# manuelbb-upb/Morbit.jl

Hardware: AMD Instinct MI355X
Metric: RBF build+solve+eval cycles/sec (higher is better)
Workload: dtype f64

## Files before the change

### morbit.jl_amd/csrc/backsolve.hip

```cpp
#include "common.hpp"

namespace mrbf {

namespace bsolve {

constexpr int NB = 128, NTHR = 512;
typedef double v2d __attribute__((ext_vector_type(2)));
typedef double v4d __attribute__((ext_vector_type(4)));
typedef __attribute__((address_space(1))) unsigned gu32;
typedef __attribute__((address_space(1))) double gf64;
typedef __attribute__((address_space(1))) v2d gv2d;

template <int KB>
struct Shared {
    double xs[2][KB][NB];
    int ok;
};

__global__ __launch_bounds__(256) void premul_kernel(const double *__restrict__ L, int64_t lda, const double *__restrict__ linv_all,
                                                     double *__restrict__ Mbuf, int nb, unsigned *__restrict__ flags, int nflags,
                                                     unsigned long long *__restrict__ xb, int nxb) {
    for (int e = blockIdx.x * 256 + threadIdx.x; e < nflags; e += gridDim.x * 256) flags[e] = 0u;
    for (int e = blockIdx.x * 256 + threadIdx.x; e < nxb; e += gridDim.x * 256) xb[e] = ~0ull;
    const int slab = blockIdx.x & 3, t = (blockIdx.x >> 2) & 1, j = blockIdx.x >> 3;
    const int i = j + 1 + t;
    if (i >= nb) return;
    const double *A = L + (int64_t)i * NB + (int64_t)j * NB * lda;
    const double *B = linv_all + (size_t)j * NB * NB;
    double *M = Mbuf + ((size_t)j * 2 + t) * NB * NB;
    const int lane = threadIdx.x & 63, wave = threadIdx.x >> 6, l15 = lane & 15, l4 = lane >> 4;
    const int i0 = 32 * wave, j0 = 32 * slab;
    v4d acc[2][2];
#pragma unroll
    for (int a = 0; a < 2; ++a)
#pragma unroll
        for (int b = 0; b < 2; ++b) acc[a][b] = (v4d){0.0, 0.0, 0.0, 0.0};
    const double *pa = A + (i0 + l15) + (int64_t)(j0 + l4) * lda;
    const double *pb = B + (j0 + l4) + (int64_t)(j0 + l15) * NB;
    constexpr int UK = 8;
    double fa0[2][UK], fa1[2][UK], fb0[2][UK], fb1[2][UK];
    auto burst = [&](int buf) {
#pragma unroll
        for (int u = 0; u < UK; ++u) {
            fa0[buf][u] = pa[(int64_t)4 * u * lda];
            fa1[buf][u] = pa[(int64_t)4 * u * lda + 16];
            fb0[buf][u] = pb[4 * u];
            fb1[buf][u] = pb[4 * u + 16 * NB];
        }
        pa += (int64_t)4 * UK * lda;
        pb += 4 * UK;
    };
    auto mma = [&](int buf) {
#pragma unroll
        for (int u = 0; u < UK; ++u) {
            acc[0][0] = __builtin_amdgcn_mfma_f64_16x16x4f64(fa0[buf][u], fb0[buf][u], acc[0][0], 0, 0, 0);
            acc[0][1] = __builtin_amdgcn_mfma_f64_16x16x4f64(fa0[buf][u], fb1[buf][u], acc[0][1], 0, 0, 0);
            acc[1][0] = __builtin_amdgcn_mfma_f64_16x16x4f64(fa1[buf][u], fb0[buf][u], acc[1][0], 0, 0, 0);
            acc[1][1] = __builtin_amdgcn_mfma_f64_16x16x4f64(fa1[buf][u], fb1[buf][u], acc[1][1], 0, 0, 0);
        }
    };
    const int nburst = (NB - j0) / (4 * UK);
    burst(0);
    for (int b = 0; b < nburst; b += 2) {
        if (b + 1 < nburst) burst(1);
        mma(0);
        if (b + 1 >= nburst) break;
        if (b + 2 < nburst) burst(0);
        mma(1);
    }
#pragma unroll
    for (int a = 0; a < 2; ++a)
#pragma unroll
        for (int b = 0; b < 2; ++b)
#pragma unroll
            for (int r = 0; r < 4; ++r) M[(i0 + 16 * a + l4 + 4 * r) + (size_t)(j0 + 16 * b + l15) * NB] = acc[a][b][r];
}

__device__ __forceinline__ void load_tile(const double *__restrict__ T, int64_t ldt, v2d (&r)[2][8]) {
    const int lane = threadIdx.x & 63, w = threadIdx.x >> 6;
    const double *p = T + (int64_t)(16 * w + 2 * (lane >> 3)) * ldt + 2 * (lane & 7);
#pragma unroll
    for (int cc = 0; cc < 2; ++cc)
#pragma unroll
        for (int u = 0; u < 8; ++u) r[cc][u] = *(const gv2d *)(p + cc * ldt + 16 * u);
}

template <int N>
__device__ __forceinline__ double shl_lanes(double v) {
    const long long b = __double_as_longlong(v);
    const int lo = __builtin_amdgcn_update_dpp((int)b, (int)b, 0x100 + N, 0xf, 0xf, false);
    const int hi = __builtin_amdgcn_update_dpp((int)(b >> 32), (int)(b >> 32), 0x100 + N, 0xf, 0xf, false);
    return __longlong_as_double(((long long)hi << 32) | (unsigned)lo);
}

template <int KB>
__device__ __forceinline__ void tile_dot(const double (*xs)[NB], const v2d (&r)[2][8], double (&out)[2][KB]) {
    const int q = threadIdx.x & 7;
    double acc[2][KB];
#pragma unroll
    for (int cc = 0; cc < 2; ++cc)
#pragma unroll
        for (int l = 0; l < KB; ++l) acc[cc][l] = 0.0;
#pragma unroll
    for (int u = 0; u < 8; ++u) {
#pragma unroll
        for (int l = 0; l < KB; ++l) {
            const v2d x = *(const v2d *)&xs[l][16 * u + 2 * q];
#pragma unroll
// ... 202 lines not shown
    double last[2][KB];
#pragma unroll
    for (int cc = 0; cc < 2; ++cc)
#pragma unroll
        for (int l = 0; l < KB; ++l) last[cc][l] = 0.0;
    if (npm >= 1) {
        if (stamps && tid == 0) stamps[256 * 4 + j] = (long long)wall_clock64();
        await_block<KB>(sh, sh.xs[1], xb, j + 1, fillv, 0, abortw, epoch, spin_ticks, status, 0x700);
        if (stamps && tid == 0) stamps[j * 4 + 0] = (long long)wall_clock64();
        lds_barrier();
        if (!sh.ok) return;
        if (stamps && tid == 0) stamps[j * 4 + 1] = (long long)wall_clock64();
        tile_dot<KB>(sh.xs[1], tm1, last);
    } else {
        lds_barrier();
        if (!sh.ok) return;
    }
    if ((fault & 1) && j == nb / 2) return;
    if (stamps && tid == 0) stamps[j * 4 + 2] = (long long)wall_clock64();
    if (q == 0) {
#pragma unroll
        for (int l = 0; l < KB; ++l) {
            const v2d v = (v2d){(zj[l][0] - acc[0][l]) - last[0][l], (zj[l][1] - acc[1][l]) - last[1][l]};
            publish(&xb[((size_t)j * KB + l) * NB + col], v);
            *(v2d *)&Y[(int64_t)(k0 + l) * ldy + (int64_t)j * NB + col] = v;
        }
    }
}

}

int backsolve_blocked(mrbf_ctx *ctx, int64_t npad, const double *L, int64_t lda, const double *linv_all, double *Y, int64_t ldy, int k);

int backsolve_persistent(mrbf_ctx *ctx, int64_t npad, const double *L, int64_t lda, const double *linv_all, double *Y, int64_t ldy, int k,
                         int *status) {
    using namespace bsolve;
    const int nb = (int)(npad / NB);
    static const int force_old = mrbf_env("MRBF_BACKSOLVE_LAUNCHES") ? atoi(mrbf_env("MRBF_BACKSOLVE_LAUNCHES")) : 0;
    const int ncu = ctx->ncu;
    if (force_old || nb < 3 || nb > ncu || (lda & 1) || (reinterpret_cast<uintptr_t>(L) & 15))
        return backsolve_blocked(ctx, npad, L, lda, linv_all, Y, ldy, k);
    unsigned *flags;
    MRBF_TRY(get_buf(ctx, S_BSOLVE_FLAGS, (size_t)(nb + 1) * 32, &flags));
    const unsigned long long spin_ticks = (unsigned long long)std::max(1, ctx->spin_ms) * 100000ull;
    const int fault = (ctx->debug_fault & 2) ? 1 : 0;
    double *xb, *Mbuf;
    MRBF_TRY(get_buf(ctx, S_BSOLVE_X, (size_t)2 * nb * 4 * NB, &xb));
    MRBF_TRY(get_buf(ctx, S_BSOLVE_M, (size_t)nb * 2 * NB * NB, &Mbuf));
    hipLaunchKernelGGL(premul_kernel, dim3((unsigned)(8 * (nb - 1))), dim3(256), 0, ctx->stream, L, lda, linv_all, Mbuf, nb, flags, (nb + 1) * 32,
                       reinterpret_cast<unsigned long long *>(xb), 2 * nb * 4 * NB);
    static const bool want_stamps = mrbf_env("MRBF_BSOLVE_STAMPS") && atoi(mrbf_env("MRBF_BSOLVE_STAMPS")) != 0;
    long long *stamps = nullptr;
    if (want_stamps) {
        static long long *dbg = nullptr;
        if (!dbg) MRBF_HIP(ctx, hipMalloc(&dbg, (size_t)256 * 9 * sizeof(long long)));
        stamps = dbg;
    }
    unsigned epoch = 0;
    for (int k0 = 0; k0 < k; k0 += 4) {
        const int kb = std::min(4, k - k0);
        ++epoch;
        if (k0 > 0) MRBF_HIP(ctx, hipMemsetAsync(xb, 0xff, (size_t)2 * nb * 4 * NB * sizeof(double), ctx->stream));
#define MRBF_BSP(KBV)                                                                                                          \
    hipLaunchKernelGGL((backsolve_persistent_kernel<KBV>), dim3((unsigned)(2 * nb)), dim3(NTHR), 0, ctx->stream, L, lda, linv_all, Mbuf, Y, ldy, k0, nb, \
                       flags, epoch, spin_ticks, status, fault, xb, xb + (size_t)nb * 4 * NB, stamps)
        if (kb == 1) MRBF_BSP(1); else if (kb == 2) MRBF_BSP(2); else if (kb == 3) MRBF_BSP(3); else MRBF_BSP(4);
#undef MRBF_BSP
    }
    MRBF_HIP(ctx, hipGetLastError());
    if (want_stamps) {
        std::vector<long long> h((size_t)256 * 9);
        MRBF_HIP(ctx, hipMemcpyAsync(h.data(), stamps, h.size() * sizeof(long long), hipMemcpyDeviceToHost, ctx->stream));
        MRBF_HIP(ctx, hipStreamSynchronize(ctx->stream));
        double seen = 0, bar = 0, dot = 0, hop = 0, late = 0;
        int cnt = 0;
        for (int j = 1; j + 2 < nb; ++j) {
            seen += (double)(h[j * 4 + 0] - h[(j + 1) * 4 + 2]);
            bar += (double)(h[j * 4 + 1] - h[j * 4 + 0]);
            dot += (double)(h[j * 4 + 2] - h[j * 4 + 1]);
            hop += (double)(h[j * 4 + 2] - h[(j + 1) * 4 + 2]);
            late += (double)(h[256 * 4 + j] - h[(j + 1) * 4 + 2]);
            ++cnt;
        }
// ... 21 lines not shown
```

### morbit.jl_amd/csrc/chol_mega.hip

```cpp
#include <chrono>

#include "chol_diag_core.hpp"
#include "common.hpp"
#include "mega_gemm.hpp"

namespace mrbf {

typedef double v4d __attribute__((ext_vector_type(4)));
typedef double v2d __attribute__((ext_vector_type(2)));

namespace mega {

constexpr int WIN_DEFAULT = 4;

enum { JOB_U = 0, JOB_T = 1, JOB_P = 2, JOB_S = 3, JOB_UH = 4 };
struct Job {
    short kind, i, c, w;
};
enum { CTL_QP = 0, CTL_ABORT = 32, CTL_TIMEOUT = 64, CTL_PCOLS = 96, CTL_QC = 128, CTL_TS = 144 , CTL_WORDS = 160 };
constexpr int QSTRIDE = 32;
__host__ __device__ inline int wstart(int w, int first, int win) { return w <= 0 ? 0 : first + win * (w - 1); }
__host__ __device__ inline int nbulk_updates(int i, int c, int slack, int slack_chain, int first, int win, int srows = 2) {
    const int t = c - ((i - c <= srows) ? slack_chain : slack);
    return t < first ? 0 : (t - first) / win + 1;
}

struct Edge {
    int head, tail_c0, srows_edge, pstream_edge;
    int shalf, sh_head, sh_tail_c0;
    int tfull1;
    int xhalf;
};
__host__ __device__ inline bool edge_col(int c, const Edge &e) { return c < e.head || c >= e.tail_c0; }
__host__ __device__ inline int srows_at(int c, int srows, const Edge &e) { return edge_col(c, e) ? e.srows_edge : srows; }
__host__ __device__ inline bool shalf_at(int c, int srows, const Edge &e) { return e.shalf && (c < e.sh_head || c >= e.sh_tail_c0) && srows_at(c, srows, e) >= 5; }
__host__ __device__ inline bool tfull_at(int i, int c, int srows, const Edge &e) { return e.tfull1 > 0 && i - c - srows_at(c, srows, e) > e.tfull1 - 1; }
__host__ __device__ inline bool xhalf_at(int i, int nt, const Edge &e) { return e.xhalf && i >= nt; }

struct Args {
    double *A;
    int64_t lda;
    int NT, MT;
    double *linv;
    unsigned *tdone;
    unsigned *ucnt;
    unsigned *ctl;
    const Job *pjobs;
    int npanel;
    const Job *bjobs;
    int nbulk;
    const int *wq_start;
    unsigned *wq_head;
    double *itg;
    unsigned *dprog;
    unsigned *sprog;
    unsigned *quiet;
    int nwin;
    int *info;
    const Job *cjobs;
    int nchainjobs;
    int nchain;
    int ndedicated;
    int look;
    unsigned long long spin_ticks;
    int fault;
    int use_quiet;
    int xchain;
    int quiet_tail;
    int slack, slack_chain, first, win, wbias, srows;
    Edge edge;
    int cboost;
    int head_job1;
    int nreserve;
    int reserve_job0;
    unsigned long long *jlog;
    int jlog_cap;
    int pstream;
    int panel_dma;
    int trace_dbg;
    unsigned long long *trace;
};

struct Shared {
    union {
        double gemm[4 * 2 * 8 * LDS_LD];
        diagcore::DiagV6Shared diag;
    } u;
    int ok;
    int jkind, jidx;
    unsigned long long *jrec;
    int wlo;
    int cwlo;
    int mycu;
};

typedef __attribute__((address_space(1))) unsigned gu32;
typedef __attribute__((address_space(1))) double gf64;
__device__ __forceinline__ unsigned ldf(const unsigned *p) {
    return __hip_atomic_load((const gu32 *)p, __ATOMIC_RELAXED, __HIP_MEMORY_SCOPE_AGENT);
}
__device__ __forceinline__ void stf(unsigned *p, unsigned v) { __hip_atomic_store((gu32 *)p, v, __ATOMIC_RELAXED, __HIP_MEMORY_SCOPE_AGENT); }
__device__ __forceinline__ unsigned addf(unsigned *p, unsigned v) {
    return __hip_atomic_fetch_add((gu32 *)p, v, __ATOMIC_RELAXED, __HIP_MEMORY_SCOPE_AGENT);
}
__device__ __forceinline__ void st_sc1(double *p, double v) { __hip_atomic_store((gf64 *)p, v, __ATOMIC_RELAXED, __HIP_MEMORY_SCOPE_AGENT); }
__device__ __forceinline__ int64_t uni64(int64_t v) {
    const unsigned lo = (unsigned)__builtin_amdgcn_readfirstlane((int)(unsigned)(unsigned long long)v);
    const unsigned hi = (unsigned)__builtin_amdgcn_readfirstlane((int)(unsigned)((unsigned long long)v >> 32));
    return (int64_t)(((unsigned long long)hi << 32) | lo);
}
template <class T>
__device__ __forceinline__ T *uni_ptr(T *q) {
    return reinterpret_cast<T *>(uni64(reinterpret_cast<int64_t>(q)));
// ... 588 lines not shown
            }
        }
        if (has_mask == 0ull) {
            if (!moved) return -2;
            continue;
        }
        unsigned key = 0xffffffffu;
        if (has) {
            const Job jb = a.bjobs[base + (int)h];
            const int jw = jb.w & 255, pl = wstart(jw + 1, a.first, a.win) - 1;
            if (ldf(a.tdone + (size_t)jb.i * a.NT + pl) >= 2u && ldf(a.tdone + (size_t)jb.c * a.NT + pl) >= 2u &&
                ldf(a.ucnt + (size_t)jb.i * a.NT + jb.c) >= (unsigned)(2 * jw))
                key = ((unsigned)(1024 + jb.c + a.wbias * wnd - (cls ? a.cboost : 0)) << 8) | (unsigned)lane;
        }
        unsigned best = key;
#pragma unroll
        for (int off = 32; off > 0; off >>= 1) {
            const unsigned o = (unsigned)__shfl_xor((int)best, off);
            best = o < best ? o : best;
        }
        if (best == 0xffffffffu) return -1;
        const int win_lane = (int)(best & 0xffu);
        int got = -1;
        if (lane == win_lane) {
            const unsigned g = addf(a.wq_head + (size_t)wq * QSTRIDE, 1u);
            if (g < (unsigned)cnt) got = base + (int)g;
        }
        got = __shfl(got, win_lane);
        if (got >= 0) return got;
    }
    return -1;
}

__device__ __forceinline__ void mega_body(const Args &a) {
    __shared__ __attribute__((aligned(16))) Shared sh;
    const int bx = (int)blockIdx.x;
    const int nx = a.xchain, cls = nx > 0 && (bx & 7) < nx;
    const int cidx = !cls ? -1 : (bx < 256 ? (bx >> 3) * nx + (bx & 7) : 32 * nx + ((bx - 256) >> 3) * nx + (bx & 7));
    const int oidx = nx == 0 ? bx - a.nchain : (cls ? -1 : (bx < 256 ? bx - ((bx >> 3) * nx + nx) : bx - 32 * nx - (((bx - 256) >> 3) * nx + nx)));
    const bool chain = nx ? (cls && cidx < a.nchain) : bx < a.nchain;
    const bool dedicated = !chain && oidx >= 0 && oidx < a.ndedicated;
    if (chain || dedicated) __builtin_amdgcn_s_setprio(2);
    if (threadIdx.x == 0) {
        sh.wlo = 0;
        sh.cwlo = 0;
        const unsigned hw = __builtin_amdgcn_s_getreg((31 << 11) | 4);
        const unsigned xcc = __builtin_amdgcn_s_getreg((31 << 11) | 20);
        sh.mycu = (int)(((xcc & 7u) << 6) | (((hw >> 13) & 3u) << 4) | ((hw >> 8) & 15u));
    }
    __syncthreads();
    unsigned *myquiet = a.quiet + (size_t)sh.mycu * QSTRIDE;
    const bool reserve = !chain && cls && cidx < a.nchain + a.nreserve;
    bool in_chain = chain;
    if (reserve && threadIdx.x == 0) {
        const unsigned qc = ldf(a.ctl + CTL_QC);
        sh.jidx = (qc < (unsigned)a.head_job1 || qc >= (unsigned)a.reserve_job0) ? 1 : 0;
    }
    if (reserve) {
        __syncthreads();
        in_chain = sh.jidx != 0;
        __syncthreads();
    }
    unsigned long long idle_t0 = 0;
    int nidle = 0;
    while (true) {
    if (in_chain) {
        if (a.use_quiet && threadIdx.x == 0) addf(myquiet, 1u);
        if (reserve) __builtin_amdgcn_s_setprio(2);
        bool leave = false;
        while (true) {
            if (threadIdx.x == 0) {
                int idx = -1;
                if (!ldf(a.ctl + CTL_ABORT)) {
                    if (reserve) {
                        const unsigned qc = ldf(a.ctl + CTL_QC);
                        if (qc >= (unsigned)a.head_job1 && qc < (unsigned)a.reserve_job0) idx = -2;
                    }
                    if (idx != -2) {
                        const unsigned got = addf(a.ctl + CTL_QC, 1u);
                        if (got < (unsigned)a.nchainjobs) idx = (int)got;
                    }
                }
                sh.jidx = idx;
            }
            __syncthreads();
            const int idx = sh.jidx;
            __syncthreads();
            if (idx == -2) {
                leave = true;
                break;
            }
            if (idx < 0) break;
            const Job jb = a.cjobs[idx];
            jlog_begin(a, sh, jb);
            if (!(jb.kind == JOB_P ? (a.trace ? run_diag<true>(a, sh, jb) : run_diag<false>(a, sh, jb))
                                   : (jb.w == 0 ? run_stream<false>(a, sh, jb) : run_stream<true>(a, sh, jb))))
                break;
            jlog_end(sh);
        }
        if (a.use_quiet && threadIdx.x == 0) addf(myquiet, 0xffffffffu);
        if (!leave) return;
        __builtin_amdgcn_s_setprio(0);
        in_chain = false;
        idle_t0 = 0;
        nidle = 0;
        continue;
    }
    {
        if (threadIdx.x < 64) {
            int kind = -1, idx = 0;
            bool panel_left = false;
            if (ldf(a.ctl + CTL_ABORT)) {
                kind = -2;
            } else if (reserve && ldf(a.ctl + CTL_QC) >= (unsigned)a.reserve_job0 && ldf(a.ctl + CTL_QC) < (unsigned)a.nchainjobs) {
                kind = -3;
            } else if (!dedicated && a.use_quiet && ldf(myquiet) != 0 && a.NT - (int)ldf(a.ctl + CTL_PCOLS) <= a.quiet_tail) {
                kind = -1;
                idle_t0 = 0;
            } else {
                const unsigned ph = ldf(a.ctl + CTL_QP);
                panel_left = ph < (unsigned)a.npanel;
                bool want_panel = false;
                if (panel_left) {
                    if (dedicated || a.ndedicated == 0)
                        want_panel = true;
                    else {
                        const Job hj = a.pjobs[ph];
                        want_panel = hj.c < (int)ldf(a.ctl + CTL_PCOLS) + a.look &&
                                     ldf(a.ucnt + (size_t)hj.i * a.NT + hj.c) >=
                                         2u * (unsigned)nbulk_updates(hj.i, hj.c, a.slack, a.slack_chain, a.first, a.win, srows_at(hj.c, a.srows, a.edge));
                    }
                }
                if (want_panel) {
                    unsigned got = 0;
// ... 36 lines not shown
        __syncthreads();
        if (kind == -2) break;
        if (kind == -3) {
            in_chain = true;
            continue;
        }
        if (kind == -1) {
            ++nidle;
            const int reps = nidle < 8 ? 1 : (nidle < 32 ? 4 : 16);
            for (int r = 0; r < reps; ++r) __builtin_amdgcn_s_sleep(64);
            continue;
        }
        idle_t0 = 0;
        nidle = 0;
        bool ok;
        const unsigned long long tj0 = a.trace ? wall_clock64() : 0ull;
        jlog_begin(a, sh, kind == 1 ? a.pjobs[idx] : a.bjobs[idx]);
        if (kind == 1) {
            if (!dedicated) __builtin_amdgcn_s_setprio(1);
            ok = a.pjobs[idx].w == 2 ? run_panel<true>(a, sh, a.pjobs[idx]) : run_panel<false>(a, sh, a.pjobs[idx]);
            if (!dedicated) __builtin_amdgcn_s_setprio(0);
        } else {
            ok = a.bjobs[idx].kind == JOB_UH ? run_bulk<64>(a, sh, a.bjobs[idx]) : run_bulk<128>(a, sh, a.bjobs[idx]);
        }
        jlog_end(sh);
        if (a.trace && threadIdx.x == 0) {
            unsigned long long *u = a.trace + (size_t)a.NT * 16 + (size_t)blockIdx.x * 4;
            u[kind == 1 ? 1 : 0] += wall_clock64() - tj0;
            u[kind == 1 ? 3 : 2] += 1;
        }
        if (!ok) break;
    }
    }
}

__global__ __launch_bounds__(256, 2) void potrf_mega_kernel(const Args a) {
    if (threadIdx.x == 0)
        __hip_atomic_fetch_max((unsigned long long *)(a.ctl + CTL_TS), ~(unsigned long long)wall_clock64(), __ATOMIC_RELAXED, __HIP_MEMORY_SCOPE_AGENT);
    mega_body(a);
    if (threadIdx.x == 0)
        __hip_atomic_fetch_max((unsigned long long *)(a.ctl + CTL_TS + 2), (unsigned long long)wall_clock64(), __ATOMIC_RELAXED, __HIP_MEMORY_SCOPE_AGENT);
}

__global__ void mega_status_kernel(const unsigned *ctl, int *info, unsigned long long *stat) {
    if (ctl[CTL_TIMEOUT] != 0 && *info == 0) *info = -(int)ctl[CTL_TIMEOUT];
    const unsigned long long *ts = (const unsigned long long *)(ctl + CTL_TS);
    if (stat) stat[0] = (ts[0] != 0 && ts[1] != 0) ? ts[1] - ~ts[0] : 0ull;
}

}

static void build_job_tables(int NT, int MT, int slack, int slack_chain, int first, int win, int srows, const mega::Edge &edge, int half_cols,
                             int tail_half, int tail_half_w, bool chainq, std::vector<mega::Job> &pj, std::vector<mega::Job> &bj, std::vector<mega::Job> &cj, std::vector<int> &wqs) {
    using namespace mega;
    pj.clear();
    bj.clear();
    cj.clear();
    wqs.clear();
    for (int c = 0; c < NT; ++c) {
        cj.push_back(Job{JOB_P, (short)c, (short)c, (short)0});
        for (int i = c + 1; i < MT; ++i) {
            if (i <= c + srows_at(c, srows, edge)) {
                if (shalf_at(c, srows, edge)) {
                    cj.push_back(Job{JOB_S, (short)i, (short)c, (short)1});
                    cj.push_back(Job{JOB_S, (short)i, (short)c, (short)2});
                } else {
// ... 197 lines not shown
            if (c < NT) job += 1 + (shalf_at(c, srows, edge) ? 2 : 1) * std::min(srows_at(c, srows, edge), MT - 1 - c);
        }
        a.nreserve = (e_head > 0 || e_tail_c0 < NT) ? (env_reserve >= 0 ? env_reserve : 12) : 0;
    }
    {
        static const int env_pdma = mrbf_env("MRBF_MEGA_PANELDMA") ? atoi(mrbf_env("MRBF_MEGA_PANELDMA")) : 1;
        a.panel_dma = env_pdma;
    }
    a.pstream = ctx->mega_pstream > 0 ? std::min(ctx->mega_pstream, srows) : (NTq <= 48 && srows >= 2 ? 2 : 1);
    a.spin_ticks = (unsigned long long)std::max(1, ctx->spin_ms) * 100000ull;
    a.fault = (ctx->debug_fault & 1) && MT > 1;
    const int grid = (NT <= 16 && ctx->mega_grid > 256) ? 256 : ctx->mega_grid;
    if (a.nchain < 1) a.nchain = 1;
    if (a.nchain + a.ndedicated >= grid) a.ndedicated = std::max(0, grid / 2 - a.nchain);
    {
        static const int env_xc = mrbf_env("MRBF_MEGA_XCHAIN") ? atoi(mrbf_env("MRBF_MEGA_XCHAIN")) : -1;
        const int xc = env_xc >= 0 ? env_xc : (a.nchain > 48 ? 4 : (a.nchain > 32 ? 2 : 1));
        a.xchain = (xc > 0 && 8 * a.nchain <= std::min(xc, 8) * grid) ? std::min(xc, 8) : 0;
        static const int qt = mrbf_env("MRBF_MEGA_QUIET_TAIL") ? atoi(mrbf_env("MRBF_MEGA_QUIET_TAIL")) : -1;
        a.quiet_tail = qt >= 0 ? qt : (NTq > 96 ? 32 : 1 << 20);
    }
    const char *trace_path = mrbf_env("MRBF_MEGA_TRACE");
    if (trace_path) {
        a.trace_dbg = mrbf_env("MRBF_MEGA_TRACE_WAVE") ? 12 + 16 * (atoi(mrbf_env("MRBF_MEGA_TRACE_WAVE")) & 3) : 4;
        MRBF_TRY(get_buf(ctx, S_MEGA_TRACE, (size_t)NT * 80 + 4 * 1024, &a.trace));
        MRBF_HIP(ctx, hipMemsetAsync(a.trace, 0, ((size_t)NT * 80 + 4 * 1024) * sizeof(unsigned long long), ctx->stream));
    }
    const char *jlog_path = mrbf_env("MRBF_MEGA_JLOG");
    if (jlog_path) {
        a.jlog_cap = ctx->mega_npanel + ctx->mega_nbulk + ctx->mega_nchainjobs + 16;
        MRBF_TRY(get_buf(ctx, S_MEGA_JLOG, (size_t)8 * a.jlog_cap + 16, &a.jlog));
        MRBF_HIP(ctx, hipMemsetAsync(a.jlog, 0, ((size_t)8 * a.jlog_cap + 16) * sizeof(unsigned long long), ctx->stream));
    }
    hipLaunchKernelGGL(potrf_mega_kernel, dim3((unsigned)grid), dim3(256), 0, ctx->stream, a);
    hnow();
    if (jlog_path) {
        std::vector<unsigned long long> h((size_t)8 * a.jlog_cap + 16);
        MRBF_HIP(ctx, hipStreamSynchronize(ctx->stream));
        MRBF_HIP(ctx, hipMemcpy(h.data(), a.jlog, h.size() * sizeof(unsigned long long), hipMemcpyDeviceToHost));
        if (FILE *f = fopen(jlog_path, "w")) {
            const unsigned long long n = std::min<unsigned long long>(h[0], (unsigned long long)a.jlog_cap);
            unsigned long long t0 = ~0ull;
            for (unsigned long long j = 0; j < n; ++j) t0 = std::min(t0, h[8 + 8 * j + 1]);
            for (unsigned long long j = 0; j < n; ++j) {
                const unsigned long long *r = &h[8 + 8 * j];
                fprintf(f, "%llu %llu %llu %llu %llu", r[0] & 0xff, (r[0] >> 8) & 0xffff, (r[0] >> 24) & 0xffff, (r[0] >> 40) & 0xfff, r[0] >> 52);
                for (int k = 1; k < 8; ++k) fprintf(f, " %.2f", r[k] ? (double)(r[k] - t0) * 0.01 : -1.0);
                fprintf(f, "\n");
            }
            fclose(f);
        }
    }
    MRBF_HIP(ctx, hipGetLastError());
    if (trace_path) {
        std::vector<unsigned long long> h((size_t)NT * 2 * 8);
        MRBF_HIP(ctx, hipStreamSynchronize(ctx->stream));
        MRBF_HIP(ctx, hipMemcpy(h.data(), a.trace, h.size() * sizeof(unsigned long long), hipMemcpyDeviceToHost));
        if (FILE *f = fopen(trace_path, "w")) {
            const unsigned long long t0 = h[0];
            for (int c = 0; c < NT; ++c) {
                fprintf(f, "%d", c);
                for (int k = 0; k < 8; ++k) fprintf(f, " %.2f", h[(size_t)c * 16 + k] ? (double)(h[(size_t)c * 16 + k] - t0) * 0.01 : -1.0);
                for (int k = 8; k < 15; ++k) fprintf(f, " %.0f", (double)h[(size_t)c * 16 + k]);
                fprintf(f, " %.2f", h[(size_t)c * 16 + 15] ? (double)(h[(size_t)c * 16 + 15] - t0) * 0.01 : -1.0);
                fprintf(f, "\n");
            }
// ... 157 lines not shown
```

### morbit.jl_amd/csrc/common.hpp

```cpp
#pragma once
#include <hip/hip_runtime.h>
#include <rocblas/rocblas.h>
#include <rocsolver/rocsolver.h>

#include <cmath>
#include <cstdlib>
#include <cstdint>
#include <cstdio>
#include <cstring>
#include <map>
#include <string>
#include <vector>

#include "../../include/mrbf.h"

namespace mrbf {

struct KP {
    int kid;
    double a, b;
    double a2;
    double sgn;
    int fast;
    int ik;
// ... 30 lines not shown
    int device = 0;
    int ncu = 256;
    hipStream_t own_stream = nullptr;
    hipStream_t stream = nullptr;
    rocblas_handle blas = nullptr;
    mrbf::Buf slots[mrbf::S_NSLOTS];
    hipEvent_t ev[8] = {};
    hipStream_t panel_stream = nullptr;
    hipEvent_t evx[4] = {};
    hipStream_t bulk_stream = nullptr;
    int bulk_masked = 0;
    int bulk_grid = 384;
    int mega_nt = 0, mega_mt = 0, mega_npanel = 0, mega_nbulk = 0, mega_nwin = 0, mega_nchainjobs = 0;
    int mega_grid = 512, mega_dedicated = 64, mega_look = 2, mega_min = 256, mega_max = 32768, mega_quiet = 1, mega_chain = 0, mega_slack = 3, mega_slack_chain = 0, mega_tab_slack = -1, mega_half_cols = 0, mega_first_window = 1, mega_win = 0, mega_wbias = 4, mega_pstream = 0, mega_srows = 0;
    std::string err;
    std::vector<mrbf::Buf> model_pool;
    int gram_mode = 0, residual = 1, force_path = 0, chol_impl = 0, eval_impl = 0, timing = 1, diag_impl = 0, chol_window = 0;
    int spin_ms = 1000, debug_fault = 0;
    unsigned long long *mega_stat_dev = nullptr;
    long mega_stat_shape = 0;
    int mega_stat_pending = 0;
    char *pin_base = nullptr;
    size_t pin_off = 0;
    bool pin_armed = false;
    struct PinOut {
        void *user;
        const void *pin;
        size_t bytes;
    };
    std::vector<PinOut> pin_out;
    unsigned long long *hpin = nullptr;
    int mega_info_clean = 0;
    int mega_xreal = 0;
    float last_device_ms = 0.f;
    int slow_launches = 0;
    int small_nc = 4;
    int small_cluster_ok = 0;
    int small_timeouts = 0;
    const double *eval_pre_xq = nullptr;
    int eval_population = 0;
    int eval_check_call = 0;
    int live_models = 0, live_round4 = 0;
    unsigned ps_rank_epoch = 0;
    int ps_multi_off = 0;
    std::map<long, float> mega_best_ms;
    std::vector<mrbf::MegaTables> mega_tables;
    unsigned long long mega_table_clock = 0;
};

struct mrbf_model {
    int64_t n = 0, npad = 0;
    int d = 0, dpad = 0, k = 0, q = 0, deg = -1;
    mrbf::KP kp{};
    double *C = nullptr;
    double *Xc = nullptr;
    double *sq = nullptr;
    double *mean = nullptr;
    double *W = nullptr;
    double *Wc = nullptr;
    double *lam = nullptr;
    void *block = nullptr;
    size_t block_bytes = 0;
};

namespace mrbf {

// ... 92 lines not shown
```

### morbit.jl_amd/csrc/solve.hip

```cpp
#include "common.hpp"
#include "small.hpp"

namespace mrbf {

__global__ void fit_publish_kernel(const int *__restrict__ dinfo, const double *__restrict__ scal, const unsigned long long *__restrict__ dstat,
                                   int *__restrict__ hflags, double *__restrict__ hscal, unsigned long long *__restrict__ hstat) {
    const int t = threadIdx.x;
    if (t < 4) hflags[t] = dinfo[t];
    if (t >= 4 && t < 6 && scal) hscal[t - 4] = scal[t - 4];
    if (t == 6 && dstat && hstat) hstat[0] = dstat[0];
}

__global__ void fill_saddle_kernel(const double *__restrict__ Pi, int64_t n, int q, double *__restrict__ S, int64_t N) {
    const int64_t idx = (int64_t)blockIdx.x * blockDim.x + threadIdx.x;
    const int64_t tot = n * q;
    if (idx < tot) {
        const int64_t i = idx % n;
        const int t = (int)(idx / n);
        const double v = Pi[idx];
        S[i + (n + t) * N] = v;
        S[(n + t) + i * N] = v;
    } else if (idx < tot + (int64_t)q * q) {
        const int64_t r = idx - tot;
        S[(n + r % q) + (n + r / q) * N] = 0.0;
// ... 239 lines not shown
    hipLaunchKernelGGL(rhs_from_values_kernel, dim3(nblk(N * k)), dim3(256), 0, ctx->stream, Y, n, k, B, N);
    MRBF_HIP(ctx, hipEventRecord(ctx->ev[0], ctx->stream));
    MRBF_TRY(launch_gram(ctx, ctx->gram_mode, M->C, M->Xc, M->sq, n, M->npad, M->d, M->dpad, M->kp, S, N));
    MRBF_HIP(ctx, hipEventRecord(ctx->ev[1], ctx->stream));
    MRBF_TRY(launch_poly_matrix(ctx, M->C, n, M->d, q, Pi, n));
    hipLaunchKernelGGL(fill_saddle_kernel, dim3(nblk(n * q + (int64_t)q * q)), dim3(256), 0, ctx->stream, Pi, n, q, S, N);
    MRBF_HIP(ctx, hipGetLastError());
    MRBF_BLAS(ctx, rocsolver_dgesvd(ctx->blas, rocblas_svect_all, rocblas_svect_all, (int)N, (int)N, S, (int)N, sv, U, (int)N, VT,
                                    (int)N, E, rocblas_outofplace, dinfo));
    MRBF_HIP(ctx, hipEventRecord(ctx->ev[2], ctx->stream));
    int hinfo = 0;
    MRBF_TRY(read_info(ctx, dinfo, &hinfo));
    info->factor_info = hinfo;
    info->path = MRBF_PATH_MINNORM;
    if (hinfo != 0) return fail(ctx, MRBF_ESINGULAR, "SVD of the saddle matrix did not converge (info = %d)", hinfo);
    MRBF_BLAS(ctx, rocblas_dgemm(ctx->blas, rocblas_operation_transpose, rocblas_operation_none, (int)N, k, (int)N, &one, U, (int)N,
                                 B, (int)N, &zero, T, (int)N));
    hipLaunchKernelGGL(scale_rows_pinv_kernel, dim3(nblk(N * k)), dim3(256), 0, ctx->stream, T, (int)N, k, sv);
    MRBF_BLAS(ctx, rocblas_dgemm(ctx->blas, rocblas_operation_transpose, rocblas_operation_none, (int)N, k, (int)N, &one, VT, (int)N,
                                 T, (int)N, &zero, B, (int)N));
    hipLaunchKernelGGL(scatter_solution_kernel, dim3(nblk(M->npad * k + (int64_t)q * k)), dim3(256), 0, ctx->stream, B, N, n,
                       M->npad, k, q, n, M->W, M->Wc, M->lam, B, N);
    MRBF_HIP(ctx, hipGetLastError());
    MRBF_HIP(ctx, hipEventRecord(ctx->ev[3], ctx->stream));
    MRBF_HIP(ctx, hipEventSynchronize(ctx->ev[3]));
    MRBF_HIP(ctx, hipEventElapsedTime(&info->ms_gram, ctx->ev[0], ctx->ev[1]));
    MRBF_HIP(ctx, hipEventElapsedTime(&info->ms_factor, ctx->ev[1], ctx->ev[2]));
    MRBF_HIP(ctx, hipEventElapsedTime(&info->ms_solve, ctx->ev[2], ctx->ev[3]));
    return 0;
}

int potrf_blocked_tall(mrbf_ctx *ctx, int64_t ncols, int64_t mrows, double *A, int64_t lda, int *dinfo, double *linv_all);
int backsolve_blocked(mrbf_ctx *ctx, int64_t npad, const double *L, int64_t lda, const double *linv_all, double *Y, int64_t ldy, int k);
int backsolve_persistent(mrbf_ctx *ctx, int64_t npad, const double *L, int64_t lda, const double *linv_all, double *Y, int64_t ldy, int k,
                         int *status);
int launch_update_lower(mrbf_ctx *ctx, const double *A, int64_t lda, const double *B, int64_t ldb, double *C, int64_t ldc, int64_t nt, int K,
                        const double *cvec, double cs, int64_t cn);
int launch_pad_identity(mrbf_ctx *ctx, double *A, int64_t n, int64_t npad, int64_t ld);
int tsmm_tn(mrbf_ctx *ctx, int64_t n, int p, int r, double alpha, const double *A, int64_t lda, const double *B, int64_t ldb, double beta,
            double *C, int64_t ldc);
int symm_panel(mrbf_ctx *ctx, int64_t n, int64_t npad, int q, const double *Phi, int64_t ld, const double *Q, int64_t ldq, double *W,
               int64_t ldwo, bool const_first, double cval);

__global__ void set_rhs_rows_kernel(double *__restrict__ A, int64_t ld, int64_t npad, int xt, const double *__restrict__ B, int k) {
    const int64_t idx = (int64_t)blockIdx.x * blockDim.x + threadIdx.x;
    if (idx >= npad * xt) return;
    const int l = (int)(idx % xt);
    const int64_t i = idx / xt;
    A[(npad + l) + i * ld] = (l < k) ? B[i + (int64_t)l * npad] : 0.0;
}
__global__ void get_rhs_rows_kernel(const double *__restrict__ A, int64_t ld, int64_t npad, double *__restrict__ B, int k) {
    const int64_t idx = (int64_t)blockIdx.x * blockDim.x + threadIdx.x;
    if (idx >= npad * k) return;
    const int l = (int)(idx % k);
    const int64_t i = idx / k;
    B[i + (int64_t)l * npad] = A[(npad + l) + i * ld];
}
__global__ void xc_to_tall_kernel(const double *__restrict__ Xc, int64_t n, int d, int dpad, double *__restrict__ Tall, int64_t lt,
                                  int64_t dq) {
    const int64_t idx = (int64_t)blockIdx.x * blockDim.x + threadIdx.x;
    if (idx >= n * d) return;
    const int64_t i = idx / d;
    const int t = (int)(idx % d);
    Tall[(dq + i) + (int64_t)t * lt] = Xc[i * dpad + t];
}
__global__ void build_q1_kernel(const double *__restrict__ Tall, int64_t lt, int64_t dq, int64_t n, int64_t npad, int q,
// ... 325 lines not shown
        const int K2 = (int)round_up(2 * (q - skip), 16);
        double *PA, *PB, *v0 = nullptr;
        MRBF_TRY(get_buf(ctx, S_STAGE_C, (size_t)npad * K2, &PA));
        MRBF_TRY(get_buf(ctx, S_STAGE_D, (size_t)npad * K2, &PB));
        if (skip) MRBF_TRY(get_buf(ctx, S_V0, (size_t)npad, &v0));
        MRBF_TRY(launch_projection_small(ctx, M, Wpart, rspart, nseg, LxInv, Q1, Wm, G, scal, dinfo, K2, skip, PA, PB, v0));
        MRBF_TRY(launch_update_lower(ctx, PA, npad, PB, npad, Phi, ld, npad / 128, K2, v0, 1.0 / std::sqrt((double)n), n));
    } else if (q > 0) {
        MRBF_TRY(symm_panel(ctx, n, npad, q, Phi, ld, Q1, npad, Wm, npad, true, 1.0 / std::sqrt((double)n)));
        MRBF_TRY(tsmm_tn(ctx, n, q, q, 1.0, Q1, npad, Wm, npad, 0.0, G, q));
        hipLaunchKernelGGL(trace_kernel, dim3(1), dim3(256), 0, ctx->stream, G, q, scal);
        MRBF_BLAS(ctx, rocblas_dgemm(ctx->blas, rocblas_operation_none, rocblas_operation_none, (int)n, q, q, &mhalf, Q1, (int)npad,
                                     G, q, &one, Wm, (int)npad));
        hipLaunchKernelGGL(shift_from_trace_kernel, dim3(1), dim3(1), 0, ctx->stream, scal, (double)n * M->kp.phi0,
                           (double)std::max<int64_t>(n - q, 1), dinfo);
        const int skip = (q > 1 && round_up(2 * (q - 1), 16) < round_up(2 * q, 16)) ? 1 : 0;
        const int K2 = (int)round_up(2 * (q - skip), 16);
        double *PA, *PB, *v0 = nullptr;
        MRBF_TRY(get_buf(ctx, S_STAGE_C, (size_t)npad * K2, &PA));
        MRBF_TRY(get_buf(ctx, S_STAGE_D, (size_t)npad * K2, &PB));
        if (skip) MRBF_TRY(get_buf(ctx, S_V0, (size_t)npad, &v0));
        hipLaunchKernelGGL(build_panels_kernel, dim3(nblk(npad * K2)), dim3(256), 0, ctx->stream, Q1, Wm, scal, n, npad, q, K2, skip, PA, PB, v0);
        MRBF_TRY(launch_update_lower(ctx, PA, npad, PB, npad, Phi, ld, npad / 128, K2, v0, 1.0 / std::sqrt((double)n), n));
    }
    MRBF_HIP(ctx, hipEventRecord(ctx->ev[2], ctx->stream));
    int hinfo = 0;
    double *linv_all = nullptr;
    if (builtin) {
        MRBF_TRY(get_buf(ctx, S_CHOL_WS, (size_t)npad * 128, &linv_all));
        MRBF_TRY(launch_pad_identity(ctx, Phi, n, npad, ld));
        if (q == 0) hipLaunchKernelGGL(set_rhs_rows_kernel, dim3(nblk(npad * xt)), dim3(256), 0, ctx->stream, Phi, ld, npad, xt, B, k);
        ctx->mega_xreal = k;
        ctx->mega_info_clean = 1;
        const int rc_potrf = potrf_blocked_tall(ctx, npad, npad + xt, Phi, ld, dinfo, linv_all);
        ctx->mega_xreal = 0;
        ctx->mega_info_clean = 0;
        if (rc_potrf != 0) return rc_potrf;
        MRBF_HIP(ctx, hipEventRecord(ctx->ev[3], ctx->stream));
    } else {
        int *dpot;
        MRBF_TRY(get_buf(ctx, S_IPIV, (size_t)4, &dpot));
        MRBF_BLAS(ctx, rocsolver_dpotrf(ctx->blas, rocblas_fill_lower, (int)n, Phi, (int)ld, dpot));
        MRBF_HIP(ctx, hipMemcpyAsync(dinfo, dpot, sizeof(int), hipMemcpyDeviceToDevice, ctx->stream));
        MRBF_HIP(ctx, hipEventRecord(ctx->ev[3], ctx->stream));
    }
    double *T1w = nullptr;
    if (q > 0) MRBF_TRY(get_buf(ctx, S_T1W, (size_t)q * k, &T1w));
    auto solve_tail = [&](bool persistent) -> int {
        if (builtin) {
            hipLaunchKernelGGL(get_rhs_rows_kernel, dim3(nblk(npad * k)), dim3(256), 0, ctx->stream, Phi, ld, npad, B, k);
            if (persistent)
                MRBF_TRY(backsolve_persistent(ctx, npad, Phi, ld, linv_all, B, npad, k, dinfo + 3));
            else
                MRBF_TRY(backsolve_blocked(ctx, npad, Phi, ld, linv_all, B, npad, k));
        } else {
            MRBF_BLAS(ctx, rocsolver_dpotrs(ctx->blas, rocblas_fill_lower, (int)n, k, Phi, (int)ld, B, (int)npad));
        }
        static const int tail3 = mrbf_env("MRBF_TAIL3") ? atoi(mrbf_env("MRBF_TAIL3")) : 1;
        if (tail3 && q > 0 && q <= 129 && k <= 16 && (q == 1 || LxInv)) {
            const int nch = (int)(npad / 64);
            double *T2, *part;
            MRBF_TRY(get_buf(ctx, S_T2, (size_t)q * k, &T2));
            MRBF_TRY(get_buf(ctx, S_TAIL_PART, (size_t)nch * 2 * k * q, &part));
            hipLaunchKernelGGL(tail_dots_kernel, dim3((unsigned)nch), dim3(256), 0, ctx->stream, B, npad, Q1, Wm, npad, n, q, k, part);
            hipLaunchKernelGGL(tail_coeff_kernel, dim3(1), dim3(1024), 0, ctx->stream, part, nch, q, k, q > 1 ? d : 0, T1, G, fused ? 1.0 : 0.5, LxInv,
                               std::sqrt((double)n), M->mean, T2, T1w);
            hipLaunchKernelGGL(tail_apply_kernel, dim3((unsigned)nch), dim3(256), 0, ctx->stream, B, npad, Q1, npad, T2, T1w, n, M->npad, q, k, M->W,
// ... 323 lines not shown
```

Measured before the change: 177.4.

## Fold backsolve premultiply jobs into the persistent Cholesky mega kernel

Moves the off-diagonal L·Linv premultiply tiles that the persistent backsolve needs into the tail of the Cholesky mega kernel. Workgroups claim jobs through an atomic counter once the needed tiles are marked done. Chain-exiting groups may wait on those readiness flags, while idle groups only take jobs that are already ready. The backsolve then skips its separate premul launch when the request was served. This removes a kernel launch and overlaps the premultiply with Cholesky tail work. The cost is extra request and done state in the context, extra spin-waiting inside the mega kernel, and a limit to NT of 16 or less.

```diff
diff --git a/morbit.jl_amd/csrc/backsolve.hip b/morbit.jl_amd/csrc/backsolve.hip
--- a/morbit.jl_amd/csrc/backsolve.hip
+++ b/morbit.jl_amd/csrc/backsolve.hip
@@ -1,4 +1,5 @@
 #include "common.hpp"
+#include "premul.hpp"
 
 namespace mrbf {
 
@@ -20,60 +21,7 @@
 __global__ __launch_bounds__(256) void premul_kernel(const double *__restrict__ L, int64_t lda, const double *__restrict__ linv_all,
                                                      double *__restrict__ Mbuf, int nb, unsigned *__restrict__ flags, int nflags,
                                                      unsigned long long *__restrict__ xb, int nxb) {
-    for (int e = blockIdx.x * 256 + threadIdx.x; e < nflags; e += gridDim.x * 256) flags[e] = 0u;
-    for (int e = blockIdx.x * 256 + threadIdx.x; e < nxb; e += gridDim.x * 256) xb[e] = ~0ull;
-    const int slab = blockIdx.x & 3, t = (blockIdx.x >> 2) & 1, j = blockIdx.x >> 3;
-    const int i = j + 1 + t;
-    if (i >= nb) return;
-    const double *A = L + (int64_t)i * NB + (int64_t)j * NB * lda;
-    const double *B = linv_all + (size_t)j * NB * NB;
-    double *M = Mbuf + ((size_t)j * 2 + t) * NB * NB;
-    const int lane = threadIdx.x & 63, wave = threadIdx.x >> 6, l15 = lane & 15, l4 = lane >> 4;
-    const int i0 = 32 * wave, j0 = 32 * slab;
-    v4d acc[2][2];
-#pragma unroll
-    for (int a = 0; a < 2; ++a)
-#pragma unroll
-        for (int b = 0; b < 2; ++b) acc[a][b] = (v4d){0.0, 0.0, 0.0, 0.0};
-    const double *pa = A + (i0 + l15) + (int64_t)(j0 + l4) * lda;
-    const double *pb = B + (j0 + l4) + (int64_t)(j0 + l15) * NB;
-    constexpr int UK = 8;
-    double fa0[2][UK], fa1[2][UK], fb0[2][UK], fb1[2][UK];
-    auto burst = [&](int buf) {
-#pragma unroll
-        for (int u = 0; u < UK; ++u) {
-            fa0[buf][u] = pa[(int64_t)4 * u * lda];
-            fa1[buf][u] = pa[(int64_t)4 * u * lda + 16];
-            fb0[buf][u] = pb[4 * u];
-            fb1[buf][u] = pb[4 * u + 16 * NB];
-        }
-        pa += (int64_t)4 * UK * lda;
-        pb += 4 * UK;
-    };
-    auto mma = [&](int buf) {
-#pragma unroll
-        for (int u = 0; u < UK; ++u) {
-            acc[0][0] = __builtin_amdgcn_mfma_f64_16x16x4f64(fa0[buf][u], fb0[buf][u], acc[0][0], 0, 0, 0);
-            acc[0][1] = __builtin_amdgcn_mfma_f64_16x16x4f64(fa0[buf][u], fb1[buf][u], acc[0][1], 0, 0, 0);
-            acc[1][0] = __builtin_amdgcn_mfma_f64_16x16x4f64(fa1[buf][u], fb0[buf][u], acc[1][0], 0, 0, 0);
-            acc[1][1] = __builtin_amdgcn_mfma_f64_16x16x4f64(fa1[buf][u], fb1[buf][u], acc[1][1], 0, 0, 0);
-        }
-    };
-    const int nburst = (NB - j0) / (4 * UK);
-    burst(0);
-    for (int b = 0; b < nburst; b += 2) {
-        if (b + 1 < nburst) burst(1);
-        mma(0);
-        if (b + 1 >= nburst) break;
-        if (b + 2 < nburst) burst(0);
-        mma(1);
-    }
-#pragma unroll
-    for (int a = 0; a < 2; ++a)
-#pragma unroll
-        for (int b = 0; b < 2; ++b)
-#pragma unroll
-            for (int r = 0; r < 4; ++r) M[(i0 + 16 * a + l4 + 4 * r) + (size_t)(j0 + 16 * b + l15) * NB] = acc[a][b][r];
+    premul::premul_job((int)blockIdx.x, L, lda, linv_all, Mbuf, nb, flags, nflags, xb, nxb, [](int, int) { return true; });
 }
 
 __device__ __forceinline__ void load_tile(const double *__restrict__ T, int64_t ldt, v2d (&r)[2][8]) {
@@ -342,23 +290,54 @@
 
 int backsolve_blocked(mrbf_ctx *ctx, int64_t npad, const double *L, int64_t lda, const double *linv_all, double *Y, int64_t ldy, int k);
 
+namespace bsolve {
+static bool persistent_path(mrbf_ctx *ctx, int nb, const double *L, int64_t lda) {
+    static const int force_old = mrbf_env("MRBF_BACKSOLVE_LAUNCHES") ? atoi(mrbf_env("MRBF_BACKSOLVE_LAUNCHES")) : 0;
+    return !(force_old || nb < 3 || nb > ctx->ncu || (lda & 1) || (reinterpret_cast<uintptr_t>(L) & 15));
+}
+static int buffers(mrbf_ctx *ctx, int nb, unsigned **flags, double **xb, double **Mbuf) {
+    MRBF_TRY(get_buf(ctx, S_BSOLVE_FLAGS, (size_t)(nb + 1) * 32, flags));
+    MRBF_TRY(get_buf(ctx, S_BSOLVE_X, (size_t)2 * nb * 4 * NB, xb));
+    MRBF_TRY(get_buf(ctx, S_BSOLVE_M, (size_t)nb * 2 * NB * NB, Mbuf));
+    return 0;
+}
+}
+
+int bsolve_premul_request(mrbf_ctx *ctx, int64_t npad, const double *L, int64_t lda, const double *linv_all) {
+    using namespace bsolve;
+    ctx->premul_req = mrbf_ctx::PremulReq{};
+    ctx->premul_done = mrbf_ctx::PremulReq{};
+    static const int env_on = mrbf_env("MRBF_MEGA_PREMUL") ? atoi(mrbf_env("MRBF_MEGA_PREMUL")) : 1;
+    const int nb = (int)(npad / NB);
+    if (!env_on || !linv_all || !persistent_path(ctx, nb, L, lda)) return 0;
+    mrbf_ctx::PremulReq r;
+    double *xb;
+    MRBF_TRY(buffers(ctx, nb, &r.flags, &xb, &r.M));
+    r.xb = reinterpret_cast<unsigned long long *>(xb);
+    r.L = L;
+    r.linv = linv_all;
+    r.lda = lda;
+    r.nb = nb;
+    ctx->premul_req = r;
+    return 0;
+}
+
 int backsolve_persistent(mrbf_ctx *ctx, int64_t npad, const double *L, int64_t lda, const double *linv_all, double *Y, int64_t ldy, int k,
                          int *status) {
     using namespace bsolve;
     const int nb = (int)(npad / NB);
-    static const int force_old = mrbf_env("MRBF_BACKSOLVE_LAUNCHES") ? atoi(mrbf_env("MRBF_BACKSOLVE_LAUNCHES")) : 0;
-    const int ncu = ctx->ncu;
-    if (force_old || nb < 3 || nb > ncu || (lda & 1) || (reinterpret_cast<uintptr_t>(L) & 15))
-        return backsolve_blocked(ctx, npad, L, lda, linv_all, Y, ldy, k);
+    const mrbf_ctx::PremulReq done = ctx->premul_done;
+    ctx->premul_done = mrbf_ctx::PremulReq{};
+    if (!persistent_path(ctx, nb, L, lda)) return backsolve_blocked(ctx, npad, L, lda, linv_all, Y, ldy, k);
     unsigned *flags;
-    MRBF_TRY(get_buf(ctx, S_BSOLVE_FLAGS, (size_t)(nb + 1) * 32, &flags));
+    double *xb, *Mbuf;
+    MRBF_TRY(buffers(ctx, nb, &flags, &xb, &Mbuf));
     const unsigned long long spin_ticks = (unsigned long long)std::max(1, ctx->spin_ms) * 100000ull;
     const int fault = (ctx->debug_fault & 2) ? 1 : 0;
-    double *xb, *Mbuf;
-    MRBF_TRY(get_buf(ctx, S_BSOLVE_X, (size_t)2 * nb * 4 * NB, &xb));
-    MRBF_TRY(get_buf(ctx, S_BSOLVE_M, (size_t)nb * 2 * NB * NB, &Mbuf));
-    hipLaunchKernelGGL(premul_kernel, dim3((unsigned)(8 * (nb - 1))), dim3(256), 0, ctx->stream, L, lda, linv_all, Mbuf, nb, flags, (nb + 1) * 32,
-                       reinterpret_cast<unsigned long long *>(xb), 2 * nb * 4 * NB);
+    if (!(done.L == L && done.linv == linv_all && done.lda == lda && done.nb == nb && done.M == Mbuf && done.flags == flags &&
+          done.xb == reinterpret_cast<unsigned long long *>(xb)))
+        hipLaunchKernelGGL(premul_kernel, dim3((unsigned)(8 * (nb - 1))), dim3(256), 0, ctx->stream, L, lda, linv_all, Mbuf, nb, flags, (nb + 1) * 32,
+                           reinterpret_cast<unsigned long long *>(xb), 2 * nb * 4 * NB);
     static const bool want_stamps = mrbf_env("MRBF_BSOLVE_STAMPS") && atoi(mrbf_env("MRBF_BSOLVE_STAMPS")) != 0;
     long long *stamps = nullptr;
     if (want_stamps) {
diff --git a/morbit.jl_amd/csrc/chol_mega.hip b/morbit.jl_amd/csrc/chol_mega.hip
--- a/morbit.jl_amd/csrc/chol_mega.hip
+++ b/morbit.jl_amd/csrc/chol_mega.hip
@@ -3,6 +3,7 @@
 #include "chol_diag_core.hpp"
 #include "common.hpp"
 #include "mega_gemm.hpp"
+#include "premul.hpp"
 
 namespace mrbf {
 
@@ -17,7 +18,7 @@
 struct Job {
     short kind, i, c, w;
 };
-enum { CTL_QP = 0, CTL_ABORT = 32, CTL_TIMEOUT = 64, CTL_PCOLS = 96, CTL_QC = 128, CTL_TS = 144 , CTL_WORDS = 160 };
+enum { CTL_QP = 0, CTL_ABORT = 32, CTL_TIMEOUT = 64, CTL_PCOLS = 96, CTL_QC = 128, CTL_TS = 144 , CTL_PM = 160, CTL_WORDS = 192 };
 constexpr int QSTRIDE = 32;
 __host__ __device__ inline int wstart(int w, int first, int win) { return w <= 0 ? 0 : first + win * (w - 1); }
 __host__ __device__ inline int nbulk_updates(int i, int c, int slack, int slack_chain, int first, int win, int srows = 2) {
@@ -79,6 +80,11 @@
     int panel_dma;
     int trace_dbg;
     unsigned long long *trace;
+    double *pm_M;
+    unsigned *pm_flags;
+    int pm_nflags;
+    unsigned long long *pm_xb;
+    int pm_nxb;
 };
 
 struct Shared {
@@ -733,6 +739,35 @@
     return -1;
 }
 
+__device__ __attribute__((noinline)) void run_premul(const Args &a, Shared &sh, bool may_wait) {
+    const int njobs = 8 * (a.NT - 1);
+    while (true) {
+        if (threadIdx.x == 0) {
+            int idx = -1;
+            unsigned h = ldf(a.ctl + CTL_PM);
+            while (h < (unsigned)njobs) {
+                const int j = (int)(h >> 3), i = j + 1 + (int)((h >> 2) & 1u);
+                if (!may_wait && !ldf(a.ctl + CTL_ABORT) && i < a.NT &&
+                    !(ldf(a.tdone + (size_t)i * a.NT + j) >= 2u && ldf(a.tdone + (size_t)j * a.NT + j) >= 2u))
+                    break;
+                if (__hip_atomic_compare_exchange_strong((gu32 *)(a.ctl + CTL_PM), &h, h + 1u, __ATOMIC_RELAXED, __ATOMIC_RELAXED,
+                                                         __HIP_MEMORY_SCOPE_AGENT)) {
+                    idx = (int)h;
+                    break;
+                }
+            }
+            sh.jidx = idx;
+        }
+        __syncthreads();
+        const int b = sh.jidx;
+        __syncthreads();
+        if (b < 0) return;
+        premul::premul_job(b, a.A, a.lda, a.linv, a.pm_M, a.NT, a.pm_flags, a.pm_nflags, a.pm_xb, a.pm_nxb, [&](int i, int j) {
+            return wg_wait(sh, a, a.tdone + (size_t)i * a.NT + j, 2u, a.tdone + (size_t)j * a.NT + j, 2u, nullptr, 0, 0x800u);
+        });
+    }
+}
+
 __device__ __forceinline__ void mega_body(const Args &a) {
     __shared__ __attribute__((aligned(16))) Shared sh;
     const int bx = (int)blockIdx.x;
@@ -764,6 +799,7 @@
     }
     unsigned long long idle_t0 = 0;
     int nidle = 0;
+    bool chain_exit = false;
     while (true) {
     if (in_chain) {
         if (a.use_quiet && threadIdx.x == 0) addf(myquiet, 1u);
@@ -800,7 +836,10 @@
             jlog_end(sh);
         }
         if (a.use_quiet && threadIdx.x == 0) addf(myquiet, 0xffffffffu);
-        if (!leave) return;
+        if (!leave) {
+            chain_exit = true;
+            break;
+        }
         __builtin_amdgcn_s_setprio(0);
         in_chain = false;
         idle_t0 = 0;
@@ -903,6 +942,7 @@
         if (!ok) break;
     }
     }
+    if (a.pm_M) run_premul(a, sh, chain_exit);
 }
 
 __global__ __launch_bounds__(256, 2) void potrf_mega_kernel(const Args a) {
@@ -1166,6 +1206,18 @@
         MRBF_TRY(get_buf(ctx, S_MEGA_JLOG, (size_t)8 * a.jlog_cap + 16, &a.jlog));
         MRBF_HIP(ctx, hipMemsetAsync(a.jlog, 0, ((size_t)8 * a.jlog_cap + 16) * sizeof(unsigned long long), ctx->stream));
     }
+    {
+        const mrbf_ctx::PremulReq &r = ctx->premul_req;
+        ctx->premul_done = mrbf_ctx::PremulReq{};
+        if (r.M && r.L == A && r.lda == lda && r.linv == a.linv && r.nb == NT && NT >= 2 && NT <= 16) {
+            a.pm_M = r.M;
+            a.pm_flags = r.flags;
+            a.pm_nflags = (NT + 1) * 32;
+            a.pm_xb = r.xb;
+            a.pm_nxb = 2 * NT * 4 * NB;
+            ctx->premul_done = r;
+        }
+    }
     hipLaunchKernelGGL(potrf_mega_kernel, dim3((unsigned)grid), dim3(256), 0, ctx->stream, a);
     hnow();
     if (jlog_path) {
diff --git a/morbit.jl_amd/csrc/common.hpp b/morbit.jl_amd/csrc/common.hpp
--- a/morbit.jl_amd/csrc/common.hpp
+++ b/morbit.jl_amd/csrc/common.hpp
@@ -86,6 +86,14 @@
     unsigned long long *hpin = nullptr;
     int mega_info_clean = 0;
     int mega_xreal = 0;
+    struct PremulReq {
+        const double *L = nullptr, *linv = nullptr;
+        int64_t lda = 0;
+        int nb = 0;
+        double *M = nullptr;
+        unsigned *flags = nullptr;
+        unsigned long long *xb = nullptr;
+    } premul_req, premul_done;
     float last_device_ms = 0.f;
     int slow_launches = 0;
     int small_nc = 4;
diff --git a/morbit.jl_amd/csrc/premul.hpp b/morbit.jl_amd/csrc/premul.hpp
--- /dev/null
+++ b/morbit.jl_amd/csrc/premul.hpp
@@ -0,0 +1,76 @@
+#pragma once
+#include <hip/hip_runtime.h>
+#include <cstdint>
+
+namespace mrbf {
+namespace premul {
+
+constexpr int NB = 128;
+
+__device__ __forceinline__ void premul_tile(const double *__restrict__ A, int64_t lda, const double *__restrict__ B, double *__restrict__ M,
+                                            int slab) {
+    typedef double v4d __attribute__((ext_vector_type(4)));
+    const int lane = threadIdx.x & 63, wave = threadIdx.x >> 6, l15 = lane & 15, l4 = lane >> 4;
+    const int i0 = 32 * wave, j0 = 32 * slab;
+    v4d acc[2][2];
+#pragma unroll
+    for (int a = 0; a < 2; ++a)
+#pragma unroll
+        for (int b = 0; b < 2; ++b) acc[a][b] = (v4d){0.0, 0.0, 0.0, 0.0};
+    const double *pa = A + (i0 + l15) + (int64_t)(j0 + l4) * lda;
+    const double *pb = B + (j0 + l4) + (int64_t)(j0 + l15) * NB;
+    constexpr int UK = 8;
+    double fa0[2][UK], fa1[2][UK], fb0[2][UK], fb1[2][UK];
+    auto burst = [&](int buf) {
+#pragma unroll
+        for (int u = 0; u < UK; ++u) {
+            fa0[buf][u] = pa[(int64_t)4 * u * lda];
+            fa1[buf][u] = pa[(int64_t)4 * u * lda + 16];
+            fb0[buf][u] = pb[4 * u];
+            fb1[buf][u] = pb[4 * u + 16 * NB];
+        }
+        pa += (int64_t)4 * UK * lda;
+        pb += 4 * UK;
+    };
+    auto mma = [&](int buf) {
+#pragma unroll
+        for (int u = 0; u < UK; ++u) {
+            acc[0][0] = __builtin_amdgcn_mfma_f64_16x16x4f64(fa0[buf][u], fb0[buf][u], acc[0][0], 0, 0, 0);
+            acc[0][1] = __builtin_amdgcn_mfma_f64_16x16x4f64(fa0[buf][u], fb1[buf][u], acc[0][1], 0, 0, 0);
+            acc[1][0] = __builtin_amdgcn_mfma_f64_16x16x4f64(fa1[buf][u], fb0[buf][u], acc[1][0], 0, 0, 0);
+            acc[1][1] = __builtin_amdgcn_mfma_f64_16x16x4f64(fa1[buf][u], fb1[buf][u], acc[1][1], 0, 0, 0);
+        }
+    };
+    const int nburst = (NB - j0) / (4 * UK);
+    burst(0);
+    for (int b = 0; b < nburst; b += 2) {
+        if (b + 1 < nburst) burst(1);
+        mma(0);
+        if (b + 1 >= nburst) break;
+        if (b + 2 < nburst) burst(0);
+        mma(1);
+    }
+#pragma unroll
+    for (int a = 0; a < 2; ++a)
+#pragma unroll
+        for (int b = 0; b < 2; ++b)
+#pragma unroll
+            for (int r = 0; r < 4; ++r) M[(i0 + 16 * a + l4 + 4 * r) + (size_t)(j0 + 16 * b + l15) * NB] = acc[a][b][r];
+}
+
+template <class Ready>
+__device__ __forceinline__ void premul_job(int b, const double *__restrict__ L, int64_t lda, const double *__restrict__ linv_all,
+                                           double *__restrict__ Mbuf, int nb, unsigned *__restrict__ flags, int nflags,
+                                           unsigned long long *__restrict__ xb, int nxb, Ready ready) {
+    const int njobs = 8 * (nb - 1);
+    for (int e = b * 256 + (int)threadIdx.x; e < nflags; e += njobs * 256) flags[e] = 0u;
+    for (int e = b * 256 + (int)threadIdx.x; e < nxb; e += njobs * 256) xb[e] = ~0ull;
+    const int slab = b & 3, t = (b >> 2) & 1, j = b >> 3;
+    const int i = j + 1 + t;
+    if (i >= nb) return;
+    if (!ready(i, j)) return;
+    premul_tile(L + (int64_t)i * NB + (int64_t)j * NB * lda, lda, linv_all + (size_t)j * NB * NB, Mbuf + ((size_t)j * 2 + t) * NB * NB, slab);
+}
+
+}
+}
diff --git a/morbit.jl_amd/csrc/solve.hip b/morbit.jl_amd/csrc/solve.hip
--- a/morbit.jl_amd/csrc/solve.hip
+++ b/morbit.jl_amd/csrc/solve.hip
@@ -295,6 +295,7 @@
 
 int potrf_blocked_tall(mrbf_ctx *ctx, int64_t ncols, int64_t mrows, double *A, int64_t lda, int *dinfo, double *linv_all);
 int backsolve_blocked(mrbf_ctx *ctx, int64_t npad, const double *L, int64_t lda, const double *linv_all, double *Y, int64_t ldy, int k);
+int bsolve_premul_request(mrbf_ctx *ctx, int64_t npad, const double *L, int64_t lda, const double *linv_all);
 int backsolve_persistent(mrbf_ctx *ctx, int64_t npad, const double *L, int64_t lda, const double *linv_all, double *Y, int64_t ldy, int k,
                          int *status);
 int launch_update_lower(mrbf_ctx *ctx, const double *A, int64_t lda, const double *B, int64_t ldb, double *C, int64_t ldc, int64_t nt, int K,
@@ -686,7 +687,9 @@
         if (q == 0) hipLaunchKernelGGL(set_rhs_rows_kernel, dim3(nblk(npad * xt)), dim3(256), 0, ctx->stream, Phi, ld, npad, xt, B, k);
         ctx->mega_xreal = k;
         ctx->mega_info_clean = 1;
+        MRBF_TRY(bsolve_premul_request(ctx, npad, Phi, ld, linv_all));
         const int rc_potrf = potrf_blocked_tall(ctx, npad, npad + xt, Phi, ld, dinfo, linv_all);
+        ctx->premul_req = mrbf_ctx::PremulReq{};
         ctx->mega_xreal = 0;
         ctx->mega_info_clean = 0;
         if (rc_potrf != 0) return rc_potrf;
```

New measurement: 177.4 (median of 5 runs). No clear change (+0.1%).
